# HikariTJU/LD

Hardware: AMD Instinct MI355X
Metric: images/sec (1333x800) GFocal-R50<-R101 LD train step (higher is better)
Workload: dtype f32

## Files before the change

ld_amd/csrc/conv.hip:

```cpp
#include <hip/hip_runtime.h>
#include <type_traits>
#include <stdio.h>
#include <stdlib.h>

#include <mutex>
#include <string>
#include <unordered_map>
#include <vector>

#include "conv_common.h"
#include "conv_tune.h"

namespace {

template <int BM, int BNT, int BKT, int MODE, int KG, int WVM, int WVN>
__global__ __launch_bounds__(64 * WVM * WVN * KG) void conv_igemm_kernel(ConvK a) {
  constexpr int NT = 64 * WVM * WVN;
  constexpr int WM = BM / WVM, WN = BNT / WVN;
  constexpr int TM = WM / 32, TN = WN / 32;
  constexpr int A_PER = BKT * BM / NT;
  constexpr int B_PER = BKT * BNT / NT;
  static_assert(A_PER >= 1 && B_PER >= 1, "tile too small");
  constexpr int NBUF = 2;
  constexpr int GROUP_LDS = NBUF * BKT * (BM + BNT);
// ... 2223 lines not shown
  int best = 1;
  double best_cost = 0;
  const size_t wbytes = (size_t)c->KH * c->KW * c->Cout * c->Cin * sizeof(float);
  for (int sp = 1; sp <= 256; ++sp) {
    if (sp > 1 && sp * wbytes > ((size_t)256 << 20)) break;
    int jchunk = (J + sp - 1) / sp;
    jchunk = (jchunk + bk - 1) / bk * bk;
    if (sp > 1 && (long)(sp - 1) * jchunk >= J) continue;
    const int steps = jchunk / bk;
    if (sp > 1 && steps < 4) break;
    const long waves = (long)tiles * sp;
    const double rounds = (double)((waves + slots - 1) / slots);
    const double cost = rounds * (steps + fixed) + 1e-3 * sp;
    if (sp == 1 || cost < best_cost) {
      best = sp;
      best_cost = cost;
    }
  }
  return best;
}

struct WgCfg {
  int kind, kg, bk, splits, fused;
};

static LdTuneKey wgrad_tune_key(const ld_conv_t* c) {
  return LdTuneKey{{2, c->Cin, c->Cout, c->KH, c->KW, c->stride, c->pad, c->N * c->Pout,
                    c->num_levels, c->lv[0].Hin, c->lv[0].Win, 0, 0, 0, 0, 0, 0, 0}};
}

static int wgrad_tile_max_splits(const ld_conv_t* c, int bk) {
  const int J = c->N * c->Pout;
  const int ntaps = c->KH * c->KW;
  int by_k = J / (2 * bk);
  if (by_k < 1) by_k = 1;
  int sp = by_k < 256 ? by_k : 256;
  while (sp > 1 && ld_f32_wgrad_tile_workspace(c->Cout, c->Cin, ntaps, sp) > ((size_t)128 << 20))
    --sp;
  return sp;
}

static WgCfg wgrad_model(const ld_conv_t* c) {
  WgCfg g{0, 0, 0, 0, 0};
  if (c->Cout < 48 || c->Cin < 48) return g;
  const int J = c->N * c->Pout;
  const int ntaps = c->KH * c->KW;
// ... 3 lines not shown
      g.kind = 2;
      int sp = 256 / tiles3;
      if (sp < 1) sp = 1;
      const int mx = wgrad_tile_max_splits(c, 32);
      g.splits = sp < mx ? sp : mx;
      return g;
    }
  }
  g.kind = 1;
  g.kg = 2;
  g.bk = 64;
  const int tiles = ((c->Cout + 127) / 128) * ((c->Cin + 127) / 128) * ntaps;
  const int slots = ld_f32_wgrad_tile_slots(g.kg, g.bk);
  int sp = slots / tiles;
  if (sp < 1) sp = 1;
  const int mx = wgrad_tile_max_splits(c, g.bk);
  g.splits = sp < mx ? sp : mx;
  return g;
}

static WgCfg wgrad_pick(const ld_conv_t* c) {
  if (const char* env = getenv("LD_CONV_WGRAD_CFG")) {
    WgCfg g{0, 0, 0, 0, 0};
    if (sscanf(env, "%d,%d,%d,%d,%d", &g.kind, &g.kg, &g.bk, &g.splits, &g.fused) >= 1) {
      if (g.kind == 0) return g;
      if (g.kind == 2 && c->KH == 3 && c->KW == 3) {
        const int mx = wgrad_tile_max_splits(c, 32);
        g.splits = g.splits < 1 ? 1 : (g.splits > mx ? mx : g.splits);
        return g;
      }
      if (ld_f32_wgrad_tile_cfg_ok(g.kg, g.bk)) {
        const int mx = wgrad_tile_max_splits(c, g.bk);
        if (g.splits < 1) g.splits = 1;
        if (g.splits > mx) g.splits = mx;
        return g;
      }
    }
  }
  LdTuneCfg t;
  if (ld_tune_lookup(wgrad_tune_key(c), &t)) {
    WgCfg g{t.tm, t.tn, t.wvm, t.d, t.ks};
    if (g.kind == 0) return g;
    if (g.kind == 2 && c->KH == 3 && c->KW == 3) {
      const int mx = wgrad_tile_max_splits(c, 32);
      g.splits = g.splits < 1 ? 1 : (g.splits > mx ? mx : g.splits);
      return g;
    }
// ... 73 lines not shown
    const size_t xf = (size_t)c->N * c->Cin * c->Pin;
    const size_t yf = (size_t)c->N * c->Cout * c->Pout;
    if (xf * 4 >= (size_t)kOOB || yf * 4 >= (size_t)kOOB) return LD_EUNSUPPORTED;
    k.x_bytes = (unsigned)(xf * 4);
    k.dy_bytes = (unsigned)(yf * 4);
  }
  const int ntaps = c->KH * c->KW;
  int nslabs = k.splits;
  auto deferred = [&]() -> int {
    defer->slabs = (const float*)workspace;
    defer->splits = nslabs;
    defer->ntaps = ntaps;
    defer->Cout = c->Cout;
    defer->Cin = c->Cin;
    return 0;
  };
  if (family == 2) {
    k.x_bytes = (unsigned)((size_t)c->N * c->Cin * c->Pin * 2);
    k.dy_bytes = (unsigned)((size_t)c->N * c->Cout * c->Pout * 2);
    if (int e = ld_bf16_wgrad_c8_launch(k, stream)) return e;
  } else if (family == 1) {
    if (int e = ld_bf16_wgrad_launch(k, stream)) return e;
  } else if (const WgCfg cfg = forced ? *forced : wgrad_pick(c); cfg.kind == 1) {
    const int e = ld_f32_wgrad_tile_launch(k, cfg.kg, cfg.bk, cfg.splits, cfg.fused, dw,
                                           accumulate, workspace, workspace_bytes, stream,
                                           defer ? &nslabs : nullptr);
    return e || !defer ? e : deferred();
  } else if (cfg.kind == 2) {
    const int e = ld_f32_wgrad_tap3_launch(k, cfg.splits, dw, accumulate, workspace,
                                           workspace_bytes, stream,
                                           defer ? &nslabs : nullptr);
    return e || !defer ? e : deferred();
  } else if (wmode) {
    const int blocks = ((c->Cout + 63) / 64) * ((c->Cin + 63) / 64) * ntaps * k.splits;
    if (wmode == 32)
      LD_LAUNCH(conv_wgrad_wave_kernel<32>, dim3(blocks), dim3(64), 0,
                         stream, k);
    else
      LD_LAUNCH(conv_wgrad_wave_kernel<16>, dim3(blocks), dim3(64), 0,
                         stream, k);
  } else {
    const int blocks =
        ((c->Cout + 127) / 128) * ((c->Cin + 127) / 128) * ntaps * k.splits;
    LD_LAUNCH(conv_wgrad_kernel, dim3(blocks), dim3(kThreads), 0, stream, k);
  }
  if (defer) {
    if (hipError_t e = hipGetLastError()) return (int)e;
    return deferred();
  }
  return ld_wgrad_reduce_launch(k.slabs, k.splits, ntaps, c->Cout, c->Cin, dw,
                                accumulate, stream);
}

// ... 195 lines not shown
```

ld_amd/csrc/conv_common.h:

```cpp
#pragma once
#include <hip/hip_runtime.h>
#include <stdint.h>

#include "../../include/ld_hip.h"
#include "ld_launch.h"

struct Geo {
  int stride, pad, num_levels;
  ld_conv_level_t lv[LD_MAX_LEVELS];
};

struct ConvK {
  const float* x;
  const float* wt;
  float* y;
  const float* bias;
  const float* scale;
  const float* shift;
  const float* residual;
  int relu;
  int N, Cin, Cout, KH, KW;
  int Pin, Pout;
  int J;
  int Kpad;
// ... 16 lines not shown
  const float* x;
  const float* dy;
  float* slabs;
  int N, Cin, Cout, KH, KW;
  int Pin, Pout;
  int J, splits, jchunk;
  unsigned x_bytes, dy_bytes;
  Geo g;
};

int ld_bf16_stream_launch(int mode, const ConvK& k, hipStream_t stream);
int ld_bf16_wgrad_c8_launch(const WgradK& k, hipStream_t stream);
bool ld_bf16_wgrad_c8_tiled(int Cout, int Cin);
int ld_bf16_wgrad_c8_tile_splits(int Cout, int Cin, int ntaps, int J);
int ld_bf16_stream_tune(int mode, const ConvK& k, hipStream_t stream);
bool ld_bf16_t256_fits(const ConvK& k, int BM, int BN);
int ld_bf16_t256_launch(int mode, const ConvK& k, int BM, int BN, hipStream_t stream);
int ld_bf16_wgrad_launch(const WgradK& k, hipStream_t stream);
bool ld_bf16_wgrad_tiled(int Cout, int Cin, int Pout);
int ld_bf16_wgrad_splits(int Cout, int Cin, int ntaps, int J);
bool ld_f32_wgrad_tile_cfg_ok(int kg, int bk);
int ld_f32_wgrad_tile_slots(int kg, int bk);
size_t ld_f32_wgrad_tile_workspace(int Cout, int Cin, int ntaps, int splits);
int ld_f32_wgrad_tile_launch(const WgradK& k, int kg, int bk, int splits, int fused,
                             float* dw, int accumulate, void* workspace,
                             size_t workspace_bytes, hipStream_t stream,
                             int* slabs_only = nullptr);
int ld_f32_wgrad_tap3_launch(const WgradK& k, int splits, float* dw, int accumulate,
                             void* workspace, size_t workspace_bytes, hipStream_t stream,
                             int* slabs_only = nullptr);
int ld_wgrad_reduce_launch(const float* slabs, int splits, int ntaps, int Cout,
                           int Cin, float* dw, int accumulate, hipStream_t stream);

namespace {
typedef float floatx16 __attribute__((ext_vector_type(16)));
typedef float floatx4 __attribute__((ext_vector_type(4)));

constexpr int kThreads = 256;
constexpr int WBK = 32;
constexpr int WLD = WBK + 1;

constexpr int kKPad = 32;
inline int kpad_rows(int k) { return (k + kKPad - 1) / kKPad * kKPad; }

constexpr unsigned kOOB = 0x80000000u;

typedef __amdgpu_buffer_rsrc_t rsrc_t;

__device__ __forceinline__ rsrc_t make_rsrc(const void* p, unsigned bytes) {
  const uintptr_t u = (uintptr_t)p;
  const unsigned lo = __builtin_amdgcn_readfirstlane((unsigned)u);
  const unsigned hi = __builtin_amdgcn_readfirstlane((unsigned)(u >> 32));
  void* q = (void*)(((uintptr_t)hi << 32) | lo);
// ... 70 lines not shown
```

ld_amd/csrc/conv_wgrad.hip:

```cpp
#include <hip/hip_runtime.h>
#include <stdio.h>
#include <stdlib.h>

#include <mutex>
#include <unordered_map>

#include "conv_common.h"

namespace {

typedef float floatx2 __attribute__((ext_vector_type(2)));

struct WgradTileOut {
  float* dw;
  float* part;
  unsigned* tickets;
  int accumulate;
  int out_mode;
};

constexpr int wgrad_tile_occ(int kg, int bk) {
  const int wgs = bk == 32 ? 2 : 1;
  return wgs * kg > 4 ? 4 : wgs * kg;
}

template <int KG, int BK, bool ML, int DBG = 0>
__global__ __launch_bounds__(256 * KG, wgrad_tile_occ(KG, BK)) void conv_wgrad_tile_kernel(
    WgradK a, WgradTileOut o) {
  constexpr int TB = 128;
  constexpr int NT = 256 * KG;
  constexpr int LDA = BK + 2;
  constexpr int RPASS = NT / BK;
  constexpr int NP = TB / RPASS;
  constexpr int OPF = TB * LDA;
  constexpr int STAGE = 2 * OPF;
  constexpr int KPG = BK / KG;
  constexpr int NQ = KPG / 4;
  static_assert(NP * 2 == NQ * 4, "four staging slots per quad");
  static_assert(NQ >= 2 && NQ % 2 == 0, "fragment double buffer");
  __shared__ __attribute__((aligned(16))) float lds[2 * STAGE];
  __shared__ int s_geo[LD_MAX_LEVELS * 6];
  __shared__ unsigned s_last;

  const int t = threadIdx.x, lane = t & 63;
  const int wave = __builtin_amdgcn_readfirstlane(t >> 6);
  const int kg = wave >> 2, w4 = wave & 3;
  const int wm = w4 >> 1, wn = w4 & 1;
  const int l31 = lane & 31, lk = lane >> 5;
  const int Cin = __builtin_amdgcn_readfirstlane(a.Cin);
  const int Cout = __builtin_amdgcn_readfirstlane(a.Cout);
  const int Pin = __builtin_amdgcn_readfirstlane(a.Pin);
  const int Pout = __builtin_amdgcn_readfirstlane(a.Pout);
  const int nlev = __builtin_amdgcn_readfirstlane(a.g.num_levels);
  const int stride = __builtin_amdgcn_readfirstlane(a.g.stride);
  const int pad = __builtin_amdgcn_readfirstlane(a.g.pad);
  const int mt = (Cout + TB - 1) / TB, nt = (Cin + TB - 1) / TB;
  const int ntaps = a.KH * a.KW;
  const int ntiles = mt * nt * ntaps;
  int b = xcd_swizzle(blockIdx.x, gridDim.x);
  const int tile_id = b % ntiles;
  const int split = b / ntiles;
  const int ntile = tile_id % nt;
// ... 53 lines not shown

  float sta[NP], stb[NP];
  float sta2[NP], stb2[NP];
#pragma unroll
  for (int i = 0; i < NP; ++i) sta2[i] = stb2[i] = 0.0f;
  floatx4 sta4[NP / 4], stb4[NP / 4];
#pragma unroll
  for (int i = 0; i < NP / 4; ++i) sta4[i] = stb4[i] = floatx4{0.0f, 0.0f, 0.0f, 0.0f};
  unsigned vy = kOOB, vx = kOOB;
  const int wr0 = r0 * LDA + kq;
  const int fa0 = (wm * 64 + l31) * LDA + kg * KPG + 2 * lk;
  const int fb0 = OPF + (wn * 64 + l31) * LDA + kg * KPG + 2 * lk;

  floatx16 acc[2][2];
#pragma unroll
  for (int i = 0; i < 2; ++i)
#pragma unroll
    for (int j = 0; j < 2; ++j)
#pragma unroll
      for (int r = 0; r < 16; ++r) acc[i][j][r] = 0.0f;

  const int nsteps = (jend - jbeg + BK - 1) / BK;

  {
    decode(jbeg, vy, vx);
    unsigned sa = 0, sb = 0;
#pragma unroll
    for (int i = 0; i < NP; ++i) {
      sta[i] = buf_load(ry, vy + sa, 0);
      stb[i] = buf_load(rx, vx + sb, 0);
      sa += da;
      sb += db;
    }
#pragma unroll
    for (int i = 0; i < NP; ++i) {
      lds[wr0 + i * RPASS * LDA] = sta[i];
      lds[OPF + wr0 + i * RPASS * LDA] = stb[i];
    }
    decode(jbeg + BK, vy, vx);
    sa = 0;
    sb = 0;
#pragma unroll
    for (int i = 0; i < NP; ++i) {
      sta[i] = buf_load(ry, vy + sa, 0);
      stb[i] = buf_load(rx, vx + sb, 0);
      sa += da;
      sb += db;
    }
  }
  __syncthreads();

  for (int base = 0; base < nsteps; base += 2) {
#pragma unroll
    for (int u = 0; u < 2; ++u) {
      const int step = base + u;
      if (step >= nsteps) break;
      const float* cur = lds + u * STAGE;
      float* nxt = lds + (u ^ 1) * STAGE;
      unsigned vy2 = vy, vx2 = vx;
      if (!(DBG & 8)) decode(jbeg + (step + 2) * BK, vy2, vx2);
      floatx2 fa[2][2], fb[2][2];
#pragma unroll
      for (int i = 0; i < 2; ++i) {
        fa[0][i] = *reinterpret_cast<const floatx2*>(cur + fa0 + i * 32 * LDA);
        fb[0][i] = *reinterpret_cast<const floatx2*>(cur + fb0 + i * 32 * LDA);
      }
      unsigned sa = 0, sb = 0;
#pragma unroll
      for (int q = 0; q < NQ; ++q) {
        const int c = q & 1;
        if (q + 1 < NQ && !(DBG & 16)) {
#pragma unroll
          for (int i = 0; i < 2; ++i) {
            fa[c ^ 1][i] = *reinterpret_cast<const floatx2*>(cur + fa0 + i * 32 * LDA +
                                                            4 * (q + 1));
            fb[c ^ 1][i] = *reinterpret_cast<const floatx2*>(cur + fb0 + i * 32 * LDA +
                                                            4 * (q + 1));
          }
        }
        if constexpr ((DBG & 32) != 0) {
          constexpr int NP4 = NP / 4;
          const int row4 = t / 8, quad = t % 8;
          const bool isb = q >= NP4;
          const int i4 = isb ? q - NP4 : q;
          float* dst = nxt + (isb ? OPF : 0) + (row4 + i4 * (NT / 8)) * LDA + 4 * quad;
          floatx4& reg = isb ? stb4[i4] : sta4[i4];
          if (!(DBG & 4)) {
#pragma unroll
            for (int e = 0; e < 4; ++e) dst[e] = reg[e];
          }
          const unsigned vb = isb ? vx2 - (unsigned)(r0 * Pin + kq) * 4u +
                                        (unsigned)(row4 * Pin + 4 * quad) * 4u
                                  : vy2 - (unsigned)(r0 * Pout + kq) * 4u +
                                        (unsigned)(row4 * Pout + 4 * quad) * 4u;
          const unsigned so = (unsigned)i4 * (unsigned)(NT / 8) * (unsigned)(isb ? Pin : Pout) * 4u;
          if (!(DBG & 2))
            reg = __builtin_bit_cast(floatx4, __builtin_amdgcn_raw_buffer_load_b128(
                                                  isb ? rx : ry, vb + so, 0, 0));
        } else
#pragma unroll
        for (int h = 0; h < 2; ++h) {
          const int i = 2 * q + h;
          if (!(DBG & 4)) {
// ... 2 lines not shown
          }
          if constexpr ((DBG & 64) != 0) {
            sta[i] = sta2[i];
            stb[i] = stb2[i];
            sta2[i] = buf_load(ry, vy2 + sa, 0);
            stb2[i] = buf_load(rx, vx2 + sb, 0);
          } else if (!(DBG & 2)) {
            sta[i] = buf_load(ry, vy2 + sa, 0);
            stb[i] = buf_load(rx, (DBG & 128) ? kOOB : vx2 + sb, 0);
          }
          sa += da;
          sb += db;
        }
#pragma unroll
        for (int e = 0; e < 2; ++e)
#pragma unroll
          for (int i = 0; i < 2; ++i)
#pragma unroll
            for (int j = 0; j < 2; ++j)
              acc[i][j] = __builtin_amdgcn_mfma_f32_32x32x2f32(fa[c][i][e], fb[c][j][e],
                                                               acc[i][j], 0, 0, 0);
        __builtin_amdgcn_sched_barrier(0);
      }
      if (!(DBG & 1)) __syncthreads();
    }
  }

  if (KG > 1) {
    float* red = lds;
#pragma unroll 1
    for (int g = 1; g < KG; ++g) {
      if (kg == g) {
#pragma unroll
        for (int i = 0; i < 2; ++i)
#pragma unroll
          for (int j = 0; j < 2; ++j)
#pragma unroll
            for (int r = 0; r < 16; ++r)
              red[(w4 * 64 + (i * 2 + j) * 16 + r) * 64 + lane] = acc[i][j][r];
      }
      __syncthreads();
      if (kg == 0) {
#pragma unroll
        for (int i = 0; i < 2; ++i)
#pragma unroll
          for (int j = 0; j < 2; ++j)
// ... 112 lines not shown
      }
#pragma unroll
      for (int cc = 0; cc < CH; ++cc) {
        const int c = (c0c + cc) * KG + kg;
        const int i = c >> 3, j = (c >> 2) & 1, r4 = c & 3;
        const int ci = c0 + wn * 64 + j * 32 + l31;
        if (ci >= Cin) continue;
#pragma unroll
        for (int e = 0; e < 4; ++e) {
          const int co = m0 + wm * 64 + i * 32 + e + 8 * r4 + 4 * lk;
          if (co >= Cout) continue;
          const size_t idx = ((size_t)co * Cin + ci) * ntaps + tap;
          o.dw[idx] = o.accumulate ? o.dw[idx] + sum[cc][e] : sum[cc][e];
        }
      }
    }
  }
  if (t == 0)
    __hip_atomic_store(o.tickets + tile_id, 0u, __ATOMIC_RELAXED, __HIP_MEMORY_SCOPE_AGENT);
}

template <bool ML, int DBG = 0>
__global__ __launch_bounds__(768, 3) void conv_wgrad_tap3_kernel(WgradK a, WgradTileOut o) {
  constexpr int TB = 128, BK = 32, LDA = BK + 2;
  constexpr int DYR = 144;
  constexpr int NPX = 16, NPY = 6;
  constexpr int XOFF = DYR * LDA;
  constexpr int XIMG = TB * LDA;
  constexpr int STAGE = XOFF + 3 * XIMG;
  constexpr int NQ = BK / 4;
  __shared__ __attribute__((aligned(16))) float lds[2 * STAGE];
  __shared__ int s_geo[LD_MAX_LEVELS * 6];

  const int t = threadIdx.x, lane = t & 63;
  const int wave = __builtin_amdgcn_readfirstlane(t >> 6);
  const int g = wave >> 2, w4 = wave & 3;
  const int wm = w4 >> 1, wn = w4 & 1;
  const int l31 = lane & 31, lk = lane >> 5;
  const int Cin = __builtin_amdgcn_readfirstlane(a.Cin);
  const int Cout = __builtin_amdgcn_readfirstlane(a.Cout);
  const int Pin = __builtin_amdgcn_readfirstlane(a.Pin);
  const int Pout = __builtin_amdgcn_readfirstlane(a.Pout);
  const int nlev = __builtin_amdgcn_readfirstlane(a.g.num_levels);
  const int stride = __builtin_amdgcn_readfirstlane(a.g.stride);
  const int pad = __builtin_amdgcn_readfirstlane(a.g.pad);
  const int mt = (Cout + TB - 1) / TB, nt = (Cin + TB - 1) / TB;
  const int ntiles = mt * nt * 3;
  int b = xcd_swizzle(blockIdx.x, gridDim.x);
// ... 6 lines not shown
  const int tap = kh * 3 + kw;
  const int m0 = mtile * TB, c0 = ntile * TB;
  const int jbeg = split * a.jchunk;
  const int jend = min(a.J, jbeg + a.jchunk);

  if (ML) {
    if (t < LD_MAX_LEVELS) {
      const ld_conv_level_t lv = a.g.lv[t];
      s_geo[t * 6 + 0] = lv.Hin;
      s_geo[t * 6 + 1] = lv.Win;
      s_geo[t * 6 + 2] = lv.Hout;
      s_geo[t * 6 + 3] = lv.Wout;
      s_geo[t * 6 + 4] = lv.off_in;
      s_geo[t * 6 + 5] = lv.off_out;
    }
    __syncthreads();
  }
  const int Hin0 = __builtin_amdgcn_readfirstlane(a.g.lv[0].Hin);
  const int Win0 = __builtin_amdgcn_readfirstlane(a.g.lv[0].Win);
  const int Wout0 = __builtin_amdgcn_readfirstlane(a.g.lv[0].Wout);

  const int tl = t & 255;
  const int kq = tl & 31, r0 = tl >> 5;
  const int ry0 = r0 + 48 * g;
  const rsrc_t rx = make_rsrc(a.x, a.x_bytes);
  const rsrc_t ry = make_rsrc(a.dy, a.dy_bytes);
  const unsigned da = 8u * (unsigned)Pout * 4u, db = 8u * (unsigned)Pin * 4u;

  auto decode = [&](int j0, unsigned& vy, unsigned& vx) {
    const int j = j0 + kq;
    const int n = j / Pout, p = j - n * Pout;
    int Hin = Hin0, Win = Win0, Wout = Wout0, off_in = 0, off_out = 0;
    if (ML) {
      int l = 0;
      for (int i = 1; i < nlev; ++i)
        if (p >= s_geo[i * 6 + 5]) l = i;
      Hin = s_geo[l * 6 + 0];
      Win = s_geo[l * 6 + 1];
      Wout = s_geo[l * 6 + 3];
      off_in = s_geo[l * 6 + 4];
      off_out = s_geo[l * 6 + 5];
    }
    const int r = p - off_out;
    const int ho = r / Wout, wo = r - ho * Wout;
    const int hi = ho * stride - pad + kh, wi = wo * stride - pad + kw;
    const bool jok = j < jend;
    const bool xok = jok && hi >= 0 && hi < Hin && wi >= 0 && wi < Win;
    vy = jok ? (unsigned)((n * Cout + m0 + ry0) * Pout + p) * 4u : kOOB;
    vx = xok ? (unsigned)((n * Cin + c0 + r0) * Pin + off_in + hi * Win + wi) * 4u
             : kOOB;
  };

  float sty[NPY], stx[NPX];
  unsigned vy = kOOB, vx = kOOB;
  const int wry = ry0 * LDA + kq;
  const int wrx = XOFF + g * XIMG + r0 * LDA + kq;
  const int fa0 = (wm * 64 + l31) * LDA + 2 * lk;
  const int fb0 = XOFF + g * XIMG + (wn * 64 + l31) * LDA + 2 * lk;

  floatx16 acc[2][2];
#pragma unroll
  for (int i = 0; i < 2; ++i)
#pragma unroll
    for (int j = 0; j < 2; ++j)
#pragma unroll
      for (int r = 0; r < 16; ++r) acc[i][j][r] = 0.0f;

  const int nsteps = (jend - jbeg + BK - 1) / BK;
  {
    decode(jbeg, vy, vx);
    unsigned sa = 0, sb = 0;
#pragma unroll
    for (int i = 0; i < NPX; ++i) {
      stx[i] = buf_load(rx, vx + sb, 0);
      sb += db;
      if (i < NPY) {
        sty[i] = buf_load(ry, vy + sa, 0);
        sa += da;
      }
    }
#pragma unroll
    for (int i = 0; i < NPX; ++i) {
      lds[wrx + i * 8 * LDA] = stx[i];
      if (i < NPY) lds[wry + i * 8 * LDA] = sty[i];
    }
    decode(jbeg + BK, vy, vx);
    sa = 0;
    sb = 0;
#pragma unroll
    for (int i = 0; i < NPX; ++i) {
      stx[i] = buf_load(rx, vx + sb, 0);
      sb += db;
      if (i < NPY) {
        sty[i] = buf_load(ry, vy + sa, 0);
        sa += da;
      }
    }
  }
  __syncthreads();

  for (int base = 0; base < nsteps; base += 2) {
#pragma unroll
    for (int u = 0; u < 2; ++u) {
      const int step = base + u;
      if (step >= nsteps) break;
      const float* cur = lds + u * STAGE;
      float* nxt = lds + (u ^ 1) * STAGE;
      unsigned vy2, vx2;
      decode(jbeg + (step + 2) * BK, vy2, vx2);
      floatx2 fa[2][2], fb[2][2];
#pragma unroll
      for (int i = 0; i < 2; ++i) {
        fa[0][i] = *reinterpret_cast<const floatx2*>(cur + fa0 + i * 32 * LDA);
        fb[0][i] = *reinterpret_cast<const floatx2*>(cur + fb0 + i * 32 * LDA);
      }
      unsigned sa = 0, sb = 0;
#pragma unroll
      for (int q = 0; q < NQ; ++q) {
        const int c = q & 1;
        if (q + 1 < NQ) {
#pragma unroll
          for (int i = 0; i < 2; ++i) {
            fa[c ^ 1][i] = *reinterpret_cast<const floatx2*>(cur + fa0 + i * 32 * LDA +
                                                            4 * (q + 1));
            fb[c ^ 1][i] = *reinterpret_cast<const floatx2*>(cur + fb0 + i * 32 * LDA +
                                                            4 * (q + 1));
          }
        }
#pragma unroll
        for (int h = 0; h < 2; ++h) {
          const int i = 2 * q + h;
          nxt[wrx + i * 8 * LDA] = stx[i];
          stx[i] = buf_load(rx, (DBG == 1 && g != 0) ? kOOB : vx2 + sb, 0);
          sb += db;
        }
        if (q < NPY) {
          nxt[wry + q * 8 * LDA] = sty[q];
          sty[q] = buf_load(ry, vy2 + sa, 0);
          sa += da;
        }
#pragma unroll
        for (int e = 0; e < 2; ++e)
#pragma unroll
          for (int i = 0; i < 2; ++i)
#pragma unroll
            for (int j = 0; j < 2; ++j)
              acc[i][j] = __builtin_amdgcn_mfma_f32_32x32x2f32(fa[c][i][e], fb[c][j][e],
                                                               acc[i][j], 0, 0, 0);
        __builtin_amdgcn_sched_barrier(0);
      }
      __syncthreads();
    }
  }

  if (o.out_mode == 0) {
    float* slab = a.slabs + ((size_t)split * 9 + tap) * Cout * Cin;
#pragma unroll
    for (int j = 0; j < 2; ++j) {
      const int ci = c0 + wn * 64 + j * 32 + l31;
      if (ci >= Cin) continue;
#pragma unroll
      for (int i = 0; i < 2; ++i)
#pragma unroll
        for (int r = 0; r < 16; ++r) {
          const int co = m0 + wm * 64 + i * 32 + (r & 3) + 8 * (r >> 2) + 4 * lk;
          if (co < Cout) slab[(size_t)co * Cin + ci] = acc[i][j][r];
        }
    }
  } else {
#pragma unroll
    for (int j = 0; j < 2; ++j) {
      const int ci = c0 + wn * 64 + j * 32 + l31;
// ... 42 lines not shown
      p.base = nullptr;
      return nullptr;
    }
  }
  auto it = p.slice.find(workspace);
  size_t idx;
  if (it != p.slice.end()) {
    idx = it->second;
  } else {
    if (p.next >= kTicketPools) return nullptr;
    idx = p.next++;
    p.slice[workspace] = idx;
  }
  return p.base + idx * kTicketSlots;
}

template <int DBG>
void launch_tile_dbg(const WgradK& k, const WgradTileOut& o, int blocks, hipStream_t stream) {
  LD_LAUNCH((conv_wgrad_tile_kernel<1, 32, true, DBG>), dim3(blocks), dim3(256), 0,
                     stream, k, o);
}

template <int KG, int BK>
void launch_tile(const WgradK& k, const WgradTileOut& o, int blocks, hipStream_t stream) {
  if (KG == 1 && BK == 32) {
    const char* env = getenv("LD_ALLOW_WRONG_RESULTS") ? getenv("LD_WGRAD_DBG") : nullptr;
    if (env) {
      switch (atoi(env)) {
        case 1: return launch_tile_dbg<1>(k, o, blocks, stream);
        case 2: return launch_tile_dbg<2>(k, o, blocks, stream);
        case 4: return launch_tile_dbg<4>(k, o, blocks, stream);
        case 6: return launch_tile_dbg<6>(k, o, blocks, stream);
        case 8: return launch_tile_dbg<8>(k, o, blocks, stream);
        case 14: return launch_tile_dbg<14>(k, o, blocks, stream);
        case 15: return launch_tile_dbg<15>(k, o, blocks, stream);
        case 16: return launch_tile_dbg<16>(k, o, blocks, stream);
        case 30: return launch_tile_dbg<30>(k, o, blocks, stream);
        case 31: return launch_tile_dbg<31>(k, o, blocks, stream);
        case 32: return launch_tile_dbg<32>(k, o, blocks, stream);
        case 33: return launch_tile_dbg<33>(k, o, blocks, stream);
        case 64: return launch_tile_dbg<64>(k, o, blocks, stream);
        case 128: return launch_tile_dbg<128>(k, o, blocks, stream);
        default: break;
      }
    }
  }
  if (k.g.num_levels > 1)
    LD_LAUNCH((conv_wgrad_tile_kernel<KG, BK, true>), dim3(blocks), dim3(256 * KG),
                       0, stream, k, o);
  else
    LD_LAUNCH((conv_wgrad_tile_kernel<KG, BK, false>), dim3(blocks), dim3(256 * KG),
                       0, stream, k, o);
}

}

bool ld_f32_wgrad_tile_cfg_ok(int kg, int bk) {
  return (bk == 32 && (kg == 1 || kg == 2 || kg == 4)) || (bk == 64 && (kg == 2 || kg == 4));
}

int ld_f32_wgrad_tap3_launch(const WgradK& k_in, int splits, float* dw, int accumulate,
                             void* workspace, size_t workspace_bytes, hipStream_t stream,
                             int* slabs_only) {
  if (k_in.KH != 3 || k_in.KW != 3) return LD_EUNSUPPORTED;
  WgradK k = k_in;
  const int ntiles = ((k.Cout + 127) / 128) * ((k.Cin + 127) / 128) * 3;
  if (splits < 1) splits = 1;
  int jchunk = (k.J + splits - 1) / splits;
  jchunk = (jchunk + 31) / 32 * 32;
  splits = (k.J + jchunk - 1) / jchunk;
  k.splits = splits;
  k.jchunk = jchunk;
  if ((splits > 1 || slabs_only) &&
      workspace_bytes < (size_t)splits * 9 * k.Cout * k.Cin * sizeof(float))
    return LD_ENOSPACE;
  WgradTileOut o;
  o.dw = dw;
  o.accumulate = accumulate;
  o.part = nullptr;
  o.tickets = nullptr;
  o.out_mode = splits == 1 && !slabs_only ? 1 : 0;
  k.slabs = (float*)workspace;
  const int blocks = ntiles * splits;
  if (k.g.num_levels > 1 && getenv("LD_ALLOW_WRONG_RESULTS") && getenv("LD_WGRAD_DBG") &&
      atoi(getenv("LD_WGRAD_DBG")) == 1)
    LD_LAUNCH((conv_wgrad_tap3_kernel<true, 1>), dim3(blocks), dim3(768), 0, stream,
                       k, o);
  else if (k.g.num_levels > 1)
    LD_LAUNCH((conv_wgrad_tap3_kernel<true>), dim3(blocks), dim3(768), 0, stream, k,
                       o);
  else
    LD_LAUNCH((conv_wgrad_tap3_kernel<false>), dim3(blocks), dim3(768), 0, stream, k,
                       o);
  if (hipError_t e = hipGetLastError()) return (int)e;
  if (slabs_only) {
    *slabs_only = splits;
    return 0;
  }
  if (o.out_mode == 0)
    return ld_wgrad_reduce_launch(k.slabs, splits, 9, k.Cout, k.Cin, dw, accumulate, stream);
  return 0;
}

int ld_f32_wgrad_tile_slots(int kg, int bk) {
  const int lds = 2 * 2 * 128 * (bk + 2) * 4 + 256;
  const int by_lds = (160 * 1024) / lds;
  const int by_threads = 2048 / (256 * kg);
  int per_cu = by_lds < by_threads ? by_lds : by_threads;
  if (per_cu * kg * 4 > 16) per_cu = 16 / (kg * 4);
  if (per_cu < 1) per_cu = 1;
  return 256 * per_cu;
}

size_t ld_f32_wgrad_tile_workspace(int Cout, int Cin, int ntaps, int splits) {
  const size_t ntiles = (size_t)((Cout + 127) / 128) * ((Cin + 127) / 128) * ntaps;
  const size_t fused = (size_t)splits * ntiles * 128 * 128 * sizeof(float);
  const size_t slabs = (size_t)splits * ntaps * Cout * Cin * sizeof(float);
  return fused > slabs ? fused : slabs;
}

int ld_f32_wgrad_tile_launch(const WgradK& k_in, int kg, int bk, int splits, int fused,
                             float* dw, int accumulate, void* workspace,
                             size_t workspace_bytes, hipStream_t stream, int* slabs_only) {
  if (!ld_f32_wgrad_tile_cfg_ok(kg, bk)) return LD_EUNSUPPORTED;
  WgradK k = k_in;
  const int ntaps = k.KH * k.KW;
  const int ntiles = ((k.Cout + 127) / 128) * ((k.Cin + 127) / 128) * ntaps;
  if (splits < 1) splits = 1;
  int jchunk = (k.J + splits - 1) / splits;
  jchunk = (jchunk + bk - 1) / bk * bk;
  splits = (k.J + jchunk - 1) / jchunk;
  k.splits = splits;
  k.jchunk = jchunk;
  if (workspace_bytes < ld_f32_wgrad_tile_workspace(k.Cout, k.Cin, ntaps, splits) &&
      (splits > 1 || slabs_only))
    return LD_ENOSPACE;
  WgradTileOut o;
  o.dw = dw;
  o.accumulate = accumulate;
  o.part = (float*)workspace;
  o.tickets = nullptr;
  o.out_mode = splits == 1 && !slabs_only ? 1 : 0;
  k.slabs = (float*)workspace;
  if (splits > 1 && fused && !slabs_only && (size_t)ntiles <= kTicketSlots) {
    o.tickets = ticket_slice(workspace, stream);
    if (o.tickets) o.out_mode = 2;
  }
  const int blocks = ntiles * splits;
#define LD_WT_CASE(KG_, BK_)                                  \
  if (kg == KG_ && bk == BK_) launch_tile<KG_, BK_>(k, o, blocks, stream);
  LD_WT_CASE(1, 32)
  LD_WT_CASE(2, 32)
  LD_WT_CASE(4, 32)
  LD_WT_CASE(2, 64)
  LD_WT_CASE(4, 64)
#undef LD_WT_CASE
  if (hipError_t e = hipGetLastError()) return (int)e;
  if (slabs_only) {
    *slabs_only = splits;
    return 0;
  }
  if (o.out_mode == 0)
    return ld_wgrad_reduce_launch(k.slabs, splits, ntaps, k.Cout, k.Cin, dw, accumulate,
                                  stream);
  return 0;
}
```

Baseline: 58.97.

## Add vectorized 16-byte staging loads to f32 wgrad tile and tap3 kernels

Adds a VEC=4 path to the f32 weight-gradient tile and tap3 kernels. Staging of dy and x now uses 128-bit buffer loads per quad of output pixels, with batched index decoding shared across lanes through ds_bpermute, and a scalar fix-up path for quads that cross rows, levels or padding. The path is enabled by default when stride is 1 and the widths allow it, and it is meant to cut per-element load instructions and address math. The tap3 kernel also reshapes its dy row split (DYR 144 to 128, with group 0 loading six rows and the others five). The risk is extra register pressure and fix-up overhead, plus correctness at boundaries.

```diff
diff --git a/ld_amd/csrc/conv.hip b/ld_amd/csrc/conv.hip
--- a/ld_amd/csrc/conv.hip
+++ b/ld_amd/csrc/conv.hip
@@ -2269,6 +2269,7 @@
 
 struct WgCfg {
   int kind, kg, bk, splits, fused;
+  int vec = 0;
 };
 
 static LdTuneKey wgrad_tune_key(const ld_conv_t* c) {
@@ -2318,7 +2319,9 @@
 static WgCfg wgrad_pick(const ld_conv_t* c) {
   if (const char* env = getenv("LD_CONV_WGRAD_CFG")) {
     WgCfg g{0, 0, 0, 0, 0};
-    if (sscanf(env, "%d,%d,%d,%d,%d", &g.kind, &g.kg, &g.bk, &g.splits, &g.fused) >= 1) {
+    if (sscanf(env, "%d,%d,%d,%d,%d,%d", &g.kind, &g.kg, &g.bk, &g.splits, &g.fused,
+               &g.vec) >= 1) {
+      if (g.vec != 1 && g.vec != 4) g.vec = 0;
       if (g.kind == 0) return g;
       if (g.kind == 2 && c->KH == 3 && c->KW == 3) {
         const int mx = wgrad_tile_max_splits(c, 32);
@@ -2438,13 +2441,14 @@
   } else if (family == 1) {
     if (int e = ld_bf16_wgrad_launch(k, stream)) return e;
   } else if (const WgCfg cfg = forced ? *forced : wgrad_pick(c); cfg.kind == 1) {
-    const int e = ld_f32_wgrad_tile_launch(k, cfg.kg, cfg.bk, cfg.splits, cfg.fused, dw,
-                                           accumulate, workspace, workspace_bytes, stream,
+    const int e = ld_f32_wgrad_tile_launch(k, cfg.kg, cfg.bk, cfg.splits, cfg.fused,
+                                           cfg.vec, dw, accumulate, workspace,
+                                           workspace_bytes, stream,
                                            defer ? &nslabs : nullptr);
     return e || !defer ? e : deferred();
   } else if (cfg.kind == 2) {
-    const int e = ld_f32_wgrad_tap3_launch(k, cfg.splits, dw, accumulate, workspace,
-                                           workspace_bytes, stream,
+    const int e = ld_f32_wgrad_tap3_launch(k, cfg.splits, cfg.vec, dw, accumulate,
+                                           workspace, workspace_bytes, stream,
                                            defer ? &nslabs : nullptr);
     return e || !defer ? e : deferred();
   } else if (wmode) {
diff --git a/ld_amd/csrc/conv_common.h b/ld_amd/csrc/conv_common.h
--- a/ld_amd/csrc/conv_common.h
+++ b/ld_amd/csrc/conv_common.h
@@ -62,13 +62,14 @@
 bool ld_f32_wgrad_tile_cfg_ok(int kg, int bk);
 int ld_f32_wgrad_tile_slots(int kg, int bk);
 size_t ld_f32_wgrad_tile_workspace(int Cout, int Cin, int ntaps, int splits);
+bool ld_f32_wgrad_vec4_ok(const WgradK& k);
 int ld_f32_wgrad_tile_launch(const WgradK& k, int kg, int bk, int splits, int fused,
-                             float* dw, int accumulate, void* workspace,
+                             int vec, float* dw, int accumulate, void* workspace,
                              size_t workspace_bytes, hipStream_t stream,
                              int* slabs_only = nullptr);
-int ld_f32_wgrad_tap3_launch(const WgradK& k, int splits, float* dw, int accumulate,
-                             void* workspace, size_t workspace_bytes, hipStream_t stream,
-                             int* slabs_only = nullptr);
+int ld_f32_wgrad_tap3_launch(const WgradK& k, int splits, int vec, float* dw,
+                             int accumulate, void* workspace, size_t workspace_bytes,
+                             hipStream_t stream, int* slabs_only = nullptr);
 int ld_wgrad_reduce_launch(const float* slabs, int splits, int ntaps, int Cout,
                            int Cin, float* dw, int accumulate, hipStream_t stream);
 
diff --git a/ld_amd/csrc/conv_wgrad.hip b/ld_amd/csrc/conv_wgrad.hip
--- a/ld_amd/csrc/conv_wgrad.hip
+++ b/ld_amd/csrc/conv_wgrad.hip
@@ -24,9 +24,189 @@
   return wgs * kg > 4 ? 4 : wgs * kg;
 }
 
+constexpr bool wgrad_tile_vec4(int kg, int bk) { return wgrad_tile_occ(kg, bk) <= 2; }
+constexpr int kVec4 = 256;
+
+struct WgFast {
+  unsigned vy, vx;
+  unsigned pk;
+};
+
+__device__ __forceinline__ unsigned wg_low(int k) {
+  return (1u << min(max(k, 0), 4)) - 1u;
+}
+__device__ __forceinline__ unsigned wg_high(int k) {
+  return (0xfu << min(max(k, 0), 4)) & 0xfu;
+}
+
+template <bool ML>
+__device__ __forceinline__ WgFast wgrad_quad(const int* s_geo, int nlev, int j, int jend,
+                                             int Pout, int Pin, int Cout, int Cin, int pad,
+                                             int kh, int kw, int Hin0, int Win0, int Wout0) {
+  const int n = j / Pout, p = j - n * Pout;
+  int Hin = Hin0, Win = Win0, Wout = Wout0, off_in = 0, off_out = 0, next = Pout;
+  if (ML) {
+    int l = 0;
+    for (int i = 1; i < nlev; ++i)
+      if (p >= s_geo[i * 6 + 5]) l = i;
+    Hin = s_geo[l * 6 + 0];
+    Win = s_geo[l * 6 + 1];
+    Wout = s_geo[l * 6 + 3];
+    off_in = s_geo[l * 6 + 4];
+    off_out = s_geo[l * 6 + 5];
+    next = l + 1 < nlev ? s_geo[(l + 1) * 6 + 5] : Pout;
+  }
+  const int r = p - off_out;
+  const int ho = r / Wout, wo = r - ho * Wout;
+  const int hi = ho - pad + kh, wi = wo - pad + kw;
+  const bool broken = p + 3 >= next;
+  const unsigned my = wg_low(jend - j);
+  const int c = Wout - wo;
+  const unsigned wrap = wg_high(c);
+  const unsigned rowok = ((unsigned)hi < (unsigned)Hin ? ~wrap : 0u) |
+                         ((unsigned)(hi + 1) < (unsigned)Hin ? wrap : 0u);
+  const int lo = pad - kw, hi_ = Win + pad - kw;
+  const unsigned colbad = ((wg_low(lo - wo) | wg_high(hi_ - wo)) & ~wrap) | (wg_low(lo + c) & wrap);
+  const unsigned mx = my & rowok & ~colbad;
+  WgFast f;
+  f.vy = (unsigned)(n * Cout * Pout + p) * 4u;
+  f.vx = (unsigned)(n * Cin * Pin + off_in + hi * Win + wi) * 4u;
+  f.pk = my | mx << 4 | (broken ? 0x300u : 0u);
+  return f;
+}
+
+__device__ __forceinline__ WgFast wgrad_batch_pick(const WgFast& batch, int src, unsigned yrow,
+                                                   unsigned xrow, long ysafe, long xsafe) {
+  WgFast f;
+  const unsigned vy = (unsigned)__builtin_amdgcn_ds_bpermute(src * 4, (int)batch.vy) + yrow;
+  const unsigned vx = (unsigned)__builtin_amdgcn_ds_bpermute(src * 4, (int)batch.vx) + xrow;
+  const unsigned pk = (unsigned)__builtin_amdgcn_ds_bpermute(src * 4, (int)batch.pk);
+  const bool sy = (pk & 0x100u) != 0u || (long)vy > ysafe;
+  const bool sx = (pk & 0x200u) != 0u || (long)vx > xsafe;
+  f.vy = sy ? kOOB : vy;
+  f.vx = sx ? kOOB : vx;
+  f.pk = (pk & 0xffu) | (sy ? 0x100u : 0u) | (sx ? 0x200u : 0u);
+  return f;
+}
+
+__device__ __forceinline__ long wgrad_safe(unsigned bytes, int row, int rows, int rp, int np,
+                                           unsigned pass_bytes) {
+  if (row >= rows) return 0x7fffffffffffffffL;
+  const int live = min((rows - row + rp - 1) / rp, np);
+  return (long)bytes - 16 - (long)(live - 1) * (long)pass_bytes;
+}
+
+__device__ __forceinline__ floatx4 wgrad_load4(rsrc_t r, unsigned off) {
+  return __builtin_bit_cast(floatx4, __builtin_amdgcn_raw_buffer_load_b128(r, off, 0, 0));
+}
+
+struct WgQuad {
+  unsigned vy0, vx0;
+  unsigned vy1, vx1;
+  unsigned pk;
+};
+
+template <bool ML>
+__device__ __forceinline__ WgQuad wgrad_decode4(const int* s_geo, int nlev, int j, int jend,
+                                                int Pout, int Pin, int Cout, int Cin,
+                                                int rowy, int rowx, int stride, int pad,
+                                                int kh, int kw, int Hin0, int Win0,
+                                                int Wout0) {
+  int n = j / Pout, p = j - n * Pout;
+  int l = 0;
+  if (ML) {
+    for (int i = 1; i < nlev; ++i)
+      if (p >= s_geo[i * 6 + 5]) l = i;
+  }
+  int Hin = Hin0, Win = Win0, Wout = Wout0, off_in = 0, off_out = 0, next = Pout;
+  auto geo = [&]() {
+    if (ML) {
+      Hin = s_geo[l * 6 + 0];
+      Win = s_geo[l * 6 + 1];
+      Wout = s_geo[l * 6 + 3];
+      off_in = s_geo[l * 6 + 4];
+      off_out = s_geo[l * 6 + 5];
+      next = l + 1 < nlev ? s_geo[(l + 1) * 6 + 5] : Pout;
+    }
+  };
+  geo();
+  const int r = p - off_out;
+  int ho = r / Wout, wo = r - ho * Wout;
+  unsigned pk = 0;
+  int bi = 4, ay0 = 0, ax0 = 0, ay1 = 0, ax1 = 0;
+#pragma unroll
+  for (int e = 0; e < 4; ++e) {
+    const int hi = ho * stride - pad + kh, wi = wo * stride - pad + kw;
+    const int ay = (n * Cout + rowy) * Pout + p;
+    const int ax = (n * Cin + rowx) * Pin + off_in + hi * Win + wi;
+    const bool jok = j + e < jend;
+    const bool xok = jok && hi >= 0 && hi < Hin && wi >= 0 && wi < Win;
+    pk |= (jok ? 1u : 0u) << e | (xok ? 1u : 0u) << (4 + e);
+    if (e == 0) {
+      ay0 = ay;
+      ax0 = ax;
+    } else if (bi == 4 && (ay != ay0 + e || ax != ax0 + e)) {
+      bi = e;
+      ay1 = ay;
+      ax1 = ax;
+    }
+    if (e < 3) {
+      ++p;
+      if (++wo == Wout) {
+        wo = 0;
+        ++ho;
+      }
+      if (p == next) {
+        if (p == Pout) {
+          p = 0;
+          ++n;
+          l = 0;
+        } else {
+          ++l;
+        }
+        geo();
+        ho = 0;
+        wo = 0;
+      }
+    }
+  }
+  WgQuad d;
+  d.vy0 = (unsigned)ay0 * 4u;
+  d.vx0 = (unsigned)ax0 * 4u;
+  d.vy1 = (unsigned)ay1 * 4u;
+  d.vx1 = (unsigned)ax1 * 4u;
+  d.pk = pk | (unsigned)bi << 8;
+  return d;
+}
+
+__device__ __forceinline__ void wgrad_fix4(rsrc_t r, unsigned v0, unsigned v1, unsigned pk,
+                                           int sh, unsigned s, float* dst) {
+  const unsigned bi = (pk >> 8) & 7u;
+  float v[4];
+#pragma unroll
+  for (int e = 0; e < 4; ++e) {
+    const bool ok = (pk >> (sh + e)) & 1u;
+    const unsigned a = ((unsigned)e < bi ? v0 + 4u * e : v1 + 4u * ((unsigned)e - bi)) + s;
+    v[e] = buf_load(r, ok ? a : kOOB, 0);
+  }
+#pragma unroll
+  for (int e = 0; e < 4; ++e) dst[e] = v[e];
+}
+
+__device__ __forceinline__ void wgrad_store4(float* dst, floatx4 q, unsigned pk, int sh) {
+  floatx2 lo, hi;
+  lo[0] = ((pk >> (sh + 0)) & 1u) ? q[0] : 0.0f;
+  lo[1] = ((pk >> (sh + 1)) & 1u) ? q[1] : 0.0f;
+  hi[0] = ((pk >> (sh + 2)) & 1u) ? q[2] : 0.0f;
+  hi[1] = ((pk >> (sh + 3)) & 1u) ? q[3] : 0.0f;
+  *reinterpret_cast<floatx2*>(dst) = lo;
+  *reinterpret_cast<floatx2*>(dst + 2) = hi;
+}
+
 template <int KG, int BK, bool ML, int DBG = 0>
 __global__ __launch_bounds__(256 * KG, wgrad_tile_occ(KG, BK)) void conv_wgrad_tile_kernel(
     WgradK a, WgradTileOut o) {
+  constexpr int VEC = DBG == kVec4 ? 4 : 1;
   constexpr int TB = 128;
   constexpr int NT = 256 * KG;
   constexpr int LDA = BK + 2;
@@ -36,8 +216,12 @@
   constexpr int STAGE = 2 * OPF;
   constexpr int KPG = BK / KG;
   constexpr int NQ = KPG / 4;
+  constexpr int QPR = BK / 4;
+  constexpr int RP4 = NT / QPR;
+  constexpr int NP4 = TB / RP4;
   static_assert(NP * 2 == NQ * 4, "four staging slots per quad");
   static_assert(NQ >= 2 && NQ % 2 == 0, "fragment double buffer");
+  static_assert(VEC == 1 || 2 * NP4 == NQ, "one 16-byte slot per quad");
   __shared__ __attribute__((aligned(16))) float lds[2 * STAGE];
   __shared__ int s_geo[LD_MAX_LEVELS * 6];
   __shared__ unsigned s_last;
@@ -137,6 +321,63 @@
 
   const int nsteps = (jend - jbeg + BK - 1) / BK;
 
+  const int qd = (t & 7) + (QPR == 16 ? ((t >> 4) & 1) * 8 : 0);
+  const int r4 = QPR == 16 ? ((t >> 5) << 1) + ((t >> 3) & 1) : t >> 3;
+  constexpr int SPB = 64 / QPR;
+  const unsigned da4 = (unsigned)RP4 * (unsigned)Pout * 4u;
+  const unsigned db4 = (unsigned)RP4 * (unsigned)Pin * 4u;
+  const long ysafe = wgrad_safe(a.dy_bytes, m0 + r4, Cout, RP4, NP4, da4);
+  const long xsafe = wgrad_safe(a.x_bytes, c0 + r4, Cin, RP4, NP4, db4);
+  const int wr4 = r4 * LDA + 4 * qd;
+  const unsigned yrow = (unsigned)((m0 + r4) * Pout) * 4u;
+  const unsigned xrow = (unsigned)((c0 + r4) * Pin) * 4u;
+  WgFast batch = {};
+  auto decode_batch = [&](int sl) {
+    batch = wgrad_quad<ML>(s_geo, nlev, jbeg + (sl + lane / QPR) * BK + 4 * (lane % QPR),
+                           jend, Pout, Pin, Cout, Cin, pad, kh, kw, Hin0, Win0, Wout0);
+  };
+  auto quad = [&](int sl) {
+    return wgrad_batch_pick(batch, (sl % SPB) * QPR + qd, yrow, xrow, ysafe, xsafe);
+  };
+  floatx4 qa[NP4], qb[NP4];
+  unsigned pkw = 0;
+  unsigned long fxw = 0;
+  auto fix4 = [&](int j0, unsigned pk, float* img) {
+    if (!(pk & 0x300u)) return;
+    const WgQuad d = wgrad_decode4<ML>(s_geo, nlev, j0 + 4 * qd, jend, Pout, Pin, Cout, Cin,
+                                       m0 + r4, c0 + r4, stride, pad, kh, kw, Hin0, Win0,
+                                       Wout0);
+#pragma unroll
+    for (int i = 0; i < NP4; ++i) {
+      if (pk & 0x100u)
+        wgrad_fix4(ry, d.vy0, d.vy1, d.pk, 0, i * da4, img + wr4 + i * RP4 * LDA);
+      if (pk & 0x200u)
+        wgrad_fix4(rx, d.vx0, d.vx1, d.pk, 4, i * db4, img + OPF + wr4 + i * RP4 * LDA);
+    }
+  };
+  if constexpr (VEC == 4) {
+    decode_batch(0);
+    WgFast d = quad(0);
+#pragma unroll
+    for (int i = 0; i < NP4; ++i) {
+      qa[i] = wgrad_load4(ry, d.vy + i * da4);
+      qb[i] = wgrad_load4(rx, d.vx + i * db4);
+    }
+#pragma unroll
+    for (int i = 0; i < NP4; ++i) {
+      wgrad_store4(lds + wr4 + i * RP4 * LDA, qa[i], d.pk, 0);
+      wgrad_store4(lds + OPF + wr4 + i * RP4 * LDA, qb[i], d.pk, 4);
+    }
+    if (__builtin_amdgcn_ballot_w64((d.pk & 0x300u) != 0u) != 0) fix4(jbeg, d.pk, lds);
+    d = quad(1);
+#pragma unroll
+    for (int i = 0; i < NP4; ++i) {
+      qa[i] = wgrad_load4(ry, d.vy + i * da4);
+      qb[i] = wgrad_load4(rx, d.vx + i * db4);
+    }
+    pkw = d.pk;
+    fxw = __builtin_amdgcn_ballot_w64((d.pk & 0x300u) != 0u);
+  } else
   {
     decode(jbeg, vy, vx);
     unsigned sa = 0, sb = 0;
@@ -173,7 +414,15 @@
       const float* cur = lds + u * STAGE;
       float* nxt = lds + (u ^ 1) * STAGE;
       unsigned vy2 = vy, vx2 = vx;
-      if (!(DBG & 8)) decode(jbeg + (step + 2) * BK, vy2, vx2);
+      WgFast d2 = {};
+      if constexpr (VEC == 4) {
+        if ((step + 2) % SPB == 0) {
+          asm volatile("" ::: "memory");
+          decode_batch(step + 2);
+        }
+        d2 = quad(step + 2);
+      } else if (!(DBG & 8))
+        decode(jbeg + (step + 2) * BK, vy2, vx2);
       floatx2 fa[2][2], fb[2][2];
 #pragma unroll
       for (int i = 0; i < 2; ++i) {
@@ -193,7 +442,16 @@
                                                             4 * (q + 1));
           }
         }
-        if constexpr ((DBG & 32) != 0) {
+        if constexpr (VEC == 4) {
+          if (q < NP4) {
+            wgrad_store4(nxt + wr4 + q * RP4 * LDA, qa[q], pkw, 0);
+            qa[q] = wgrad_load4(ry, d2.vy + q * da4);
+          } else {
+            const int i4 = q - NP4;
+            wgrad_store4(nxt + OPF + wr4 + i4 * RP4 * LDA, qb[i4], pkw, 4);
+            qb[i4] = wgrad_load4(rx, d2.vx + i4 * db4);
+          }
+        } else if constexpr ((DBG & 32) != 0) {
           constexpr int NP4 = NP / 4;
           const int row4 = t / 8, quad = t % 8;
           const bool isb = q >= NP4;
@@ -242,6 +500,11 @@
                                                                acc[i][j], 0, 0, 0);
         __builtin_amdgcn_sched_barrier(0);
       }
+      if constexpr (VEC == 4) {
+        if (fxw != 0) fix4(jbeg + (step + 1) * BK, pkw, nxt);
+        pkw = d2.pk;
+        fxw = __builtin_amdgcn_ballot_w64((d2.pk & 0x300u) != 0u);
+      }
       if (!(DBG & 1)) __syncthreads();
     }
   }
@@ -400,8 +663,9 @@
 
 template <bool ML, int DBG = 0>
 __global__ __launch_bounds__(768, 3) void conv_wgrad_tap3_kernel(WgradK a, WgradTileOut o) {
+  constexpr int VEC = DBG == kVec4 ? 4 : 1;
   constexpr int TB = 128, BK = 32, LDA = BK + 2;
-  constexpr int DYR = 144;
+  constexpr int DYR = 128;
   constexpr int NPX = 16, NPY = 6;
   constexpr int XOFF = DYR * LDA;
   constexpr int XIMG = TB * LDA;
@@ -454,7 +718,8 @@
 
   const int tl = t & 255;
   const int kq = tl & 31, r0 = tl >> 5;
-  const int ry0 = r0 + 48 * g;
+  const int ry0 = r0 + 8 * (5 * g + (g > 0 ? 1 : 0));
+  const bool six = g == 0;
   const rsrc_t rx = make_rsrc(a.x, a.x_bytes);
   const rsrc_t ry = make_rsrc(a.dy, a.dy_bytes);
   const unsigned da = 8u * (unsigned)Pout * 4u, db = 8u * (unsigned)Pin * 4u;
@@ -499,7 +764,63 @@
       for (int r = 0; r < 16; ++r) acc[i][j][r] = 0.0f;
 
   const int nsteps = (jend - jbeg + BK - 1) / BK;
-  {
+
+  const int qd = tl & 7, r4 = tl >> 3;
+  const unsigned db4 = 32u * (unsigned)Pin * 4u;
+  const unsigned dy96 = 96u * (unsigned)Pout * 4u;
+  const long ysafe = wgrad_safe(a.dy_bytes, m0 + 32 * g + r4, Cout, 96, six ? 2 : 1, dy96);
+  const long xsafe = wgrad_safe(a.x_bytes, c0 + r4, Cin, 32, 4, db4);
+  const int wry4 = (32 * g + r4) * LDA + 4 * qd;
+  const int wrx4 = XOFF + g * XIMG + r4 * LDA + 4 * qd;
+  const unsigned yrow = (unsigned)((m0 + 32 * g + r4) * Pout) * 4u;
+  const unsigned xrow = (unsigned)((c0 + r4) * Pin) * 4u;
+  WgFast batch = {};
+  auto decode_batch = [&](int sl) {
+    batch = wgrad_quad<ML>(s_geo, nlev, jbeg + (sl + (lane >> 3)) * BK + 4 * (lane & 7), jend,
+                           Pout, Pin, Cout, Cin, pad, kh, kw, Hin0, Win0, Wout0);
+  };
+  auto quad = [&](int sl) {
+    return wgrad_batch_pick(batch, (sl & 7) * 8 + qd, yrow, xrow, ysafe, xsafe);
+  };
+  floatx4 qx[4], qy[2];
+  unsigned pkw = 0;
+  unsigned long fxw = 0;
+  auto fix4 = [&](int j0, unsigned pk, float* img) {
+    if (!(pk & 0x300u)) return;
+    const WgQuad d = wgrad_decode4<ML>(s_geo, nlev, j0 + 4 * qd, jend, Pout, Pin, Cout, Cin,
+                                       m0 + 32 * g + r4, c0 + r4, stride, pad, kh, kw, Hin0,
+                                       Win0, Wout0);
+    if (pk & 0x200u) {
+#pragma unroll
+      for (int i = 0; i < 4; ++i)
+        wgrad_fix4(rx, d.vx0, d.vx1, d.pk, 4, i * db4, img + wrx4 + i * 32 * LDA);
+    }
+    if (pk & 0x100u) {
+      wgrad_fix4(ry, d.vy0, d.vy1, d.pk, 0, 0u, img + wry4);
+      if (six) wgrad_fix4(ry, d.vy0, d.vy1, d.pk, 0, dy96, img + wry4 + 96 * LDA);
+    }
+  };
+  auto load_y1 = [&](const WgFast& d) { return wgrad_load4(ry, six ? d.vy + dy96 : kOOB); };
+  if constexpr (VEC == 4) {
+    decode_batch(0);
+    WgFast d = quad(0);
+#pragma unroll
+    for (int i = 0; i < 4; ++i) qx[i] = wgrad_load4(rx, d.vx + i * db4);
+    qy[0] = wgrad_load4(ry, d.vy);
+    qy[1] = load_y1(d);
+#pragma unroll
+    for (int i = 0; i < 4; ++i) wgrad_store4(lds + wrx4 + i * 32 * LDA, qx[i], d.pk, 4);
+    wgrad_store4(lds + wry4, qy[0], d.pk, 0);
+    if (six) wgrad_store4(lds + wry4 + 96 * LDA, qy[1], d.pk, 0);
+    if (__builtin_amdgcn_ballot_w64((d.pk & 0x300u) != 0u) != 0) fix4(jbeg, d.pk, lds);
+    d = quad(1);
+#pragma unroll
+    for (int i = 0; i < 4; ++i) qx[i] = wgrad_load4(rx, d.vx + i * db4);
+    qy[0] = wgrad_load4(ry, d.vy);
+    qy[1] = load_y1(d);
+    pkw = d.pk;
+    fxw = __builtin_amdgcn_ballot_w64((d.pk & 0x300u) != 0u);
+  } else {
     decode(jbeg, vy, vx);
     unsigned sa = 0, sb = 0;
 #pragma unroll
@@ -507,14 +828,14 @@
       stx[i] = buf_load(rx, vx + sb, 0);
       sb += db;
       if (i < NPY) {
-        sty[i] = buf_load(ry, vy + sa, 0);
+        sty[i] = buf_load(ry, i < NPY - 1 || six ? vy + sa : kOOB, 0);
         sa += da;
       }
     }
 #pragma unroll
     for (int i = 0; i < NPX; ++i) {
       lds[wrx + i * 8 * LDA] = stx[i];
-      if (i < NPY) lds[wry + i * 8 * LDA] = sty[i];
+      if (i < NPY - 1 || (i < NPY && six)) lds[wry + i * 8 * LDA] = sty[i];
     }
     decode(jbeg + BK, vy, vx);
     sa = 0;
@@ -524,7 +845,7 @@
       stx[i] = buf_load(rx, vx + sb, 0);
       sb += db;
       if (i < NPY) {
-        sty[i] = buf_load(ry, vy + sa, 0);
+        sty[i] = buf_load(ry, i < NPY - 1 || six ? vy + sa : kOOB, 0);
         sa += da;
       }
     }
@@ -538,8 +859,16 @@
       if (step >= nsteps) break;
       const float* cur = lds + u * STAGE;
       float* nxt = lds + (u ^ 1) * STAGE;
-      unsigned vy2, vx2;
-      decode(jbeg + (step + 2) * BK, vy2, vx2);
+      unsigned vy2 = kOOB, vx2 = kOOB;
+      WgFast d2 = {};
+      if constexpr (VEC == 4) {
+        if (((step + 2) & 7) == 0) {
+          asm volatile("" ::: "memory");
+          decode_batch(step + 2);
+        }
+        d2 = quad(step + 2);
+      } else
+        decode(jbeg + (step + 2) * BK, vy2, vx2);
       floatx2 fa[2][2], fb[2][2];
 #pragma unroll
       for (int i = 0; i < 2; ++i) {
@@ -559,6 +888,18 @@
                                                             4 * (q + 1));
           }
         }
+        if constexpr (VEC == 4) {
+          if (q < 4) {
+            wgrad_store4(nxt + wrx4 + q * 32 * LDA, qx[q], pkw, 4);
+            qx[q] = wgrad_load4(rx, d2.vx + q * db4);
+          } else if (q == 4) {
+            wgrad_store4(nxt + wry4, qy[0], pkw, 0);
+            qy[0] = wgrad_load4(ry, d2.vy);
+          } else if (q == 5) {
+            if (six) wgrad_store4(nxt + wry4 + 96 * LDA, qy[1], pkw, 0);
+            qy[1] = load_y1(d2);
+          }
+        } else {
 #pragma unroll
         for (int h = 0; h < 2; ++h) {
           const int i = 2 * q + h;
@@ -567,9 +908,10 @@
           sb += db;
         }
         if (q < NPY) {
-          nxt[wry + q * 8 * LDA] = sty[q];
-          sty[q] = buf_load(ry, vy2 + sa, 0);
+          if (q < NPY - 1 || six) nxt[wry + q * 8 * LDA] = sty[q];
+          sty[q] = buf_load(ry, q < NPY - 1 || six ? vy2 + sa : kOOB, 0);
           sa += da;
+        }
         }
 #pragma unroll
         for (int e = 0; e < 2; ++e)
@@ -580,6 +922,11 @@
               acc[i][j] = __builtin_amdgcn_mfma_f32_32x32x2f32(fa[c][i][e], fb[c][j][e],
                                                                acc[i][j], 0, 0, 0);
         __builtin_amdgcn_sched_barrier(0);
+      }
+      if constexpr (VEC == 4) {
+        if (fxw != 0) fix4(jbeg + (step + 1) * BK, pkw, nxt);
+        pkw = d2.pk;
+        fxw = __builtin_amdgcn_ballot_w64((d2.pk & 0x300u) != 0u);
       }
       __syncthreads();
     }
@@ -668,7 +1015,17 @@
 }
 
 template <int KG, int BK>
-void launch_tile(const WgradK& k, const WgradTileOut& o, int blocks, hipStream_t stream) {
+void launch_tile(const WgradK& k, const WgradTileOut& o, int blocks, int vec,
+                 hipStream_t stream) {
+  if constexpr (wgrad_tile_vec4(KG, BK)) if (vec == 4) {
+    if (k.g.num_levels > 1)
+      LD_LAUNCH((conv_wgrad_tile_kernel<KG, BK, true, kVec4>), dim3(blocks), dim3(256 * KG),
+                         0, stream, k, o);
+    else
+      LD_LAUNCH((conv_wgrad_tile_kernel<KG, BK, false, kVec4>), dim3(blocks), dim3(256 * KG),
+                         0, stream, k, o);
+    return;
+  }
   if (KG == 1 && BK == 32) {
     const char* env = getenv("LD_ALLOW_WRONG_RESULTS") ? getenv("LD_WGRAD_DBG") : nullptr;
     if (env) {
@@ -701,14 +1058,28 @@
 
 }
 
+bool ld_f32_wgrad_vec4_ok(const WgradK& k) {
+  if (k.g.stride != 1 || k.x_bytes < 16u || k.dy_bytes < 16u) return false;
+  for (int l = 0; l < k.g.num_levels; ++l) {
+    const ld_conv_level_t& lv = k.g.lv[l];
+    if (lv.Wout != lv.Win || lv.Wout < 4 + k.g.pad) return false;
+  }
+  return true;
+}
+
+static int wgrad_vec(const WgradK& k, int vec) {
+  return vec != 1 && ld_f32_wgrad_vec4_ok(k) ? 4 : 1;
+}
+
 bool ld_f32_wgrad_tile_cfg_ok(int kg, int bk) {
   return (bk == 32 && (kg == 1 || kg == 2 || kg == 4)) || (bk == 64 && (kg == 2 || kg == 4));
 }
 
-int ld_f32_wgrad_tap3_launch(const WgradK& k_in, int splits, float* dw, int accumulate,
-                             void* workspace, size_t workspace_bytes, hipStream_t stream,
-                             int* slabs_only) {
+int ld_f32_wgrad_tap3_launch(const WgradK& k_in, int splits, int vec, float* dw,
+                             int accumulate, void* workspace, size_t workspace_bytes,
+                             hipStream_t stream, int* slabs_only) {
   if (k_in.KH != 3 || k_in.KW != 3) return LD_EUNSUPPORTED;
+  vec = wgrad_vec(k_in, vec);
   WgradK k = k_in;
   const int ntiles = ((k.Cout + 127) / 128) * ((k.Cin + 127) / 128) * 3;
   if (splits < 1) splits = 1;
@@ -732,6 +1103,12 @@
       atoi(getenv("LD_WGRAD_DBG")) == 1)
     LD_LAUNCH((conv_wgrad_tap3_kernel<true, 1>), dim3(blocks), dim3(768), 0, stream,
                        k, o);
+  else if (vec == 4 && k.g.num_levels > 1)
+    LD_LAUNCH((conv_wgrad_tap3_kernel<true, kVec4>), dim3(blocks), dim3(768), 0, stream,
+                       k, o);
+  else if (vec == 4)
+    LD_LAUNCH((conv_wgrad_tap3_kernel<false, kVec4>), dim3(blocks), dim3(768), 0, stream,
+                       k, o);
   else if (k.g.num_levels > 1)
     LD_LAUNCH((conv_wgrad_tap3_kernel<true>), dim3(blocks), dim3(768), 0, stream, k,
                        o);
@@ -766,9 +1143,10 @@
 }
 
 int ld_f32_wgrad_tile_launch(const WgradK& k_in, int kg, int bk, int splits, int fused,
-                             float* dw, int accumulate, void* workspace,
+                             int vec, float* dw, int accumulate, void* workspace,
                              size_t workspace_bytes, hipStream_t stream, int* slabs_only) {
   if (!ld_f32_wgrad_tile_cfg_ok(kg, bk)) return LD_EUNSUPPORTED;
+  vec = wgrad_tile_vec4(kg, bk) ? wgrad_vec(k_in, vec) : 1;
   WgradK k = k_in;
   const int ntaps = k.KH * k.KW;
   const int ntiles = ((k.Cout + 127) / 128) * ((k.Cin + 127) / 128) * ntaps;
@@ -794,7 +1172,7 @@
   }
   const int blocks = ntiles * splits;
 #define LD_WT_CASE(KG_, BK_)                                  \
-  if (kg == KG_ && bk == BK_) launch_tile<KG_, BK_>(k, o, blocks, stream);
+  if (kg == KG_ && bk == BK_) launch_tile<KG_, BK_>(k, o, blocks, vec, stream);
   LD_WT_CASE(1, 32)
   LD_WT_CASE(2, 32)
   LD_WT_CASE(4, 32)
```

After: 58.26. -1.2%, worse.
